# mrperkett/genome-kmers

Hardware: AMD Instinct MI355X
Metric: sorted 31-mers/sec end-to-end on 3.1 Gb synthetic genome; % HBM roofline (higher is better)
Workload: dtype u64

## Files before the change

genome-kmers_amd/csrc/gkm_msd.hip:

```cpp
#include <algorithm>
#include <cstdio>
#include <cstdlib>
#include <cstring>

#include "gkm_canon.h"
#include "gkm_internal.h"
#include "gkm_msd_config.h"
#include "gkm_partition.h"
#include "gkm_swar.h"

namespace gkm {

__constant__ uint8_t c_code4_msd[256];
static bool g_msd_tables = false;

static hipError_t msd_tables() {
    if (g_msd_tables) return hipSuccess;
    uint8_t code4[256] = {0};
    const char *order = "ABCDGHKMNRSTVWY";
    for (int i = 0; order[i]; ++i) code4[(uint8_t)order[i]] = (uint8_t)(i + 1);
    hipError_t e = hipMemcpyToSymbol(HIP_SYMBOL(c_code4_msd), code4, 256);
    if (e == hipSuccess) g_msd_tables = true;
    return e;
}
// ... 42 lines not shown
}

static unsigned resident_per_cu(gk_ctx *c, const void *fn, int threads) {
    auto it = c->occupancy.find({fn, threads});
    if (it != c->occupancy.end()) return (unsigned)it->second;
    int per_cu = 0;
    if (hipOccupancyMaxActiveBlocksPerMultiprocessor(&per_cu, fn, threads, 0) != hipSuccess || per_cu < 1)
        return 1;
    c->occupancy[{fn, threads}] = per_cu;
    return (unsigned)per_cu;
}


static bool no_compact() { return opt("GKM_NO_COMPACT") != nullptr; }

hipError_t launch_pack2(const uint8_t *from, uint64_t nwords, uint64_t *code, uint32_t *dol, hipStream_t s) {
    if (nwords == 0) return hipSuccess;
    hipLaunchKernelGGL(pack2_kernel<true>, dim3((unsigned)std::min<uint64_t>((nwords + 255) / 256, 65536)), dim3(256),
                       0, s, from, nwords, code, dol);
    return hipGetLastError();
}

static int pack_sequence(gk_ctx *c, const uint64_t **code, const uint32_t **dol) {
    const uint64_t nwords = (c->sba_len + kSbaPad) / 32;
    uint64_t *pc;
    uint32_t *pd;
    GK_TRY_HIP(c, scratch(c, "pk_code", nwords, &pc));
    GK_TRY_HIP(c, scratch(c, "pk_dol", nwords, &pd));
    int slot;
    timer_begin(c, "msd_pack", &slot);
    timer_units(c, slot, c->sba_len);
    hipLaunchKernelGGL(pack2_kernel<false>, dim3((unsigned)std::min<uint64_t>((nwords + 255) / 256, 65536)), dim3(256),
                       0, c->stream, c->sba, nwords, pc, pd);
    GK_TRY_HIP(c, hipGetLastError());
    timer_end(c, slot);
    *code = pc;
    *dol = pd;
    return GK_OK;
}

static const char *kLocPrefName[kLocal] = {"locp0", "locp1", "locp2", "locp3", "locp4", "locp5"};
static const char *kLocName[kLocal][2] = {{"loc0a", "loc0b"}, {"loc1a", "loc1b"}, {"loc2a", "loc2b"},
                                          {"loc3a", "loc3b"}, {"loc4a", "loc4b"}, {"loc5a", "loc5b"}};
static const char *kLocTimer[kLocal][2] = {{"msd_local_wave4", "msd_local_wave4_r"},
                                           {"msd_local_wave8", "msd_local_wave8_r"},
                                           {"msd_local_wave16", "msd_local_wave16_r"},
                                           {"msd_local_block16", "msd_local_block16_r"},
                                           {"msd_local_tiny", "msd_local_tiny_r"},
                                           {"msd_local_block32", "msd_local_block32_r"}};
static const char *kPassNames[] = {"msd_pass_l0", "msd_pass_l1", "msd_pass_l2", "msd_pass_l3",
                                   "msd_pass_l4", "msd_pass_l5", "msd_pass_l6", "msd_pass_l7"};
static const char *kPassNamesP[] = {"msd_pass_l0p", "msd_pass_l1p", "msd_pass_l2p", "msd_pass_l3p",
                                    "msd_pass_l4p", "msd_pass_l5p", "msd_pass_l6p", "msd_pass_l7p"};
static const char *kPassNamesC[] = {"msd_pass_l0c", "msd_pass_l1c", "msd_pass_l2c", "msd_pass_l3c",
                                    "msd_pass_l4c", "msd_pass_l5c", "msd_pass_l6c", "msd_pass_l7c"};

struct MsdDriver {
    gk_ctx *c;
    KeySpec ks;
    int B;
    uint64_t n = 0;
    unsigned cus, pgrid;
    int slot = -1, total_slot = -1;
    uint32_t *ctr = nullptr, h[kCtrN] = {0};
    unsigned long long *sums = nullptr, hs[kSumN] = {0};
    uint32_t *big_start[2], *big_len[2];
    uint64_t *big_pref[2];
    uint64_t *loc_pref[kLocal];
    uint32_t *dn_start, *dn_len;
    uint8_t *dn_par;
    uint2 *loc[kLocal][2];
    int wsched[kMaxLevels];
    int width(int level) const { return wsched[std::min(level, kMaxLevels - 1)]; }
    uint8_t *heads = nullptr;
    uint8_t *nd = nullptr;
    enum class Fmt { KeyStart, KeyStartDigit, Pairs, Compact, PackedL0 };
    Fmt cur_fmt = Fmt::KeyStart;
    int compact_hi = 0;
    bool allow_c79 = false;
    bool p88 = false;
    int p88_shi = 0;
    uint16_t *lo16_l0 = nullptr;
    uint8_t *nd_l0 = nullptr;
    int c79_shi = 0;
    uint16_t *lo16 = nullptr;
    uint32_t *tile_hist, *chunk_hist, *c_first, *c_ntiles, *seg_base, *seg_cnt;
    uint64_t nloc[kLocal] = {0}, loc_elems[kLocal] = {0}, ndone = 0, big_elems = 0;
    uint32_t nbig = 0;
    int cur_big = 0;
    int phase = 0;
    uint32_t ctiles = kChunkTiles;
    int wkeys = 0;
    L0Args l0a{};
    uint64_t l0_tiles = 0;

    MsdDriver(gk_ctx *c_, const KeySpec &ks_) : c(c_), ks(ks_), B(ks_.total_bits) {
        cus = cu_count(c);
        pgrid = cus * 4;
        set_widths(opt("GKM_LEVEL_BITS"));
        if (const char *e = opt("GKM_TEST_CHUNK_TILES")) ctiles = (uint32_t)std::max(1, std::atoi(e));
    }

    void enable_wide_l0() {
        const char *e = opt("GKM_WIDE_L0");
        const bool want = e && *e && std::strcmp(e, "0") != 0;
        if (want && ks.bits == 2 && !ks.canonical && !ks.acgt_only && B > kWideL0 + 8) wsched[0] = kWideL0;
    }

    void set_widths(const char *spec) {
        for (int l = 0; l < kMaxLevels; ++l) wsched[l] = kGR;
        if (ks.bits == 2) wsched[0] = 7;
        if (!spec) return;
        int l = 0, w = kGR;
        for (const char *p = spec; *p && l < kMaxLevels;) {
            w = std::min(8, std::max(6, std::atoi(p)));
            wsched[l++] = w;
            while (*p && *p != ',') ++p;
            if (*p == ',') ++p;
        }
        for (; l < kMaxLevels; ++l) wsched[l] = w;
        if (ks.bits != 2) wsched[0] = kGR;
        wsched[0] = std::max(wsched[0], ks.canonical ? 7 : 6);
    }

    Lists lists(int g, int bigsel) {
        return Lists{big_start[bigsel], big_len[bigsel], dn_start, dn_len, dn_par,
                     {loc[0][g], loc[1][g], loc[2][g], loc[3][g], loc[4][g], loc[5][g]}, big_pref[bigsel],
                     {g ? nullptr : loc_pref[0], g ? nullptr : loc_pref[1], g ? nullptr : loc_pref[2],
                      g ? nullptr : loc_pref[3], g ? nullptr : loc_pref[4], g ? nullptr : loc_pref[5]}};
    }

    int grow_done(uint64_t extra) {
        GK_TRY_HIP(c, grow_keep(c, "dn_start", ndone + extra, ndone, &dn_start));
        GK_TRY_HIP(c, grow_keep(c, "dn_len", ndone + extra, ndone, &dn_len));
        GK_TRY_HIP(c, grow_keep(c, "dn_par", ndone + extra, ndone, &dn_par));
        return GK_OK;
    }

    int init(uint64_t n_) {
        n = n_;
        GK_TRY_HIP(c, msd_tables());
        static_assert(4 * kCtrN <= 64 && 64 + 8 * kSumN <= 8 * kHostPinWords, "list counter block");
        uint64_t *cs;
        GK_TRY_HIP(c, scratch(c, "msd_ctr_sums", 8 + kSumN, &cs));
        ctr = reinterpret_cast<uint32_t *>(cs);
        sums = reinterpret_cast<unsigned long long *>(cs + 8);
        GK_TRY_HIP(c, hipMemsetAsync(ctr, 0, 4 * kCtrN, c->stream));
        const uint64_t max_big = n / kBlockMax + 2;
        GK_TRY_HIP(c, scratch(c, "big_start0", max_big, &big_start[0]));
        GK_TRY_HIP(c, scratch(c, "big_len0", max_big, &big_len[0]));
        GK_TRY_HIP(c, scratch(c, "big_start1", max_big, &big_start[1]));
        GK_TRY_HIP(c, scratch(c, "big_len1", max_big, &big_len[1]));
        GK_TRY_HIP(c, scratch(c, "big_pref0", max_big, &big_pref[0]));
        GK_TRY_HIP(c, scratch(c, "big_pref1", max_big, &big_pref[1]));
        if (int rc = grow_done(1024)) return rc;
        for (int k = 0; k < kLocal; ++k) GK_TRY_HIP(c, grow_keep(c, kLocName[k][0], 1024, 0, &loc[k][0]));
        for (int k = 0; k < kLocal; ++k) GK_TRY_HIP(c, grow_keep(c, kLocPrefName[k], 1024, 0, &loc_pref[k]));
        GK_TRY_HIP(c, scratch(c, "msd_heads", n + 64, &heads));
        return GK_OK;
    }

    int symbols_per_word() const { return 64 / ks.bits; }
    int phases() const { return (ks.symbols + symbols_per_word() - 1) / symbols_per_word(); }

    static constexpr uint64_t kInitLater = ~0ull;
    int begin(uint64_t n_, int key_bits = 0) {
        B = key_bits ? key_bits : ks.bits * std::min(ks.symbols, symbols_per_word());
// ... 314 lines not shown
    int classify(uint64_t nsub, int hi, int parity, int bigsel, const uint32_t *base = nullptr,
                 const uint32_t *cnt = nullptr, uint32_t min_size = 1, const uint64_t *ppref = nullptr, int pw = 0,
                 int compact = 0, bool read = true) {
        if (!base) base = seg_base;
        if (!cnt) cnt = seg_cnt;
        for (int k = 0; k < kLocal; ++k)
            GK_TRY_HIP(c, grow_keep(c, kLocName[k][0], nloc[k] + nsub, nloc[k], &loc[k][0]));
        for (int k = 0; k < kLocal; ++k)
            GK_TRY_HIP(c, grow_keep(c, kLocPrefName[k], nloc[k] + nsub, nloc[k], &loc_pref[k]));
        if (int rc = grow_done(nsub)) return rc;
        GK_TRY_HIP(c, hipMemsetAsync(ctr + kCtrBig, 0, 4, c->stream));
        GK_TRY_HIP(c, hipMemsetAsync(sums, 0, 8 * kSumN, c->stream));
        timer_begin(c, "msd_classify", &slot);
        hipLaunchKernelGGL(classify_kernel, dim3((unsigned)((nsub + kClassT - 1) / kClassT)), dim3(kClassT), 0,
                           c->stream, base, cnt, nsub, hi, B, parity, lists(0, bigsel), ctr, sums, min_size, ppref, pw,
                           compact, (uint32_t)kPTile, ctiles);
        GK_TRY_HIP(c, hipGetLastError());
        timer_end(c, slot);
        return read ? classify_counts() : GK_OK;
    }

    int classify_counts() {
        int r = read_ctr();
        if (r != GK_OK) return r;
        for (int k = 0; k < kLocal; ++k) {
            nloc[k] = h[kCtrLoc + k];
            loc_elems[k] += hs[kCtrLoc + k];
        }
        ndone = h[kCtrDone];
        nbig = h[kCtrBig];
        big_elems = hs[kCtrBig];
        return GK_OK;
    }

    int route_uniform(int out, uint32_t nb, bool dev_count) {
        const uint32_t *nb_dev = dev_count ? ctr + kCtrBig : nullptr;
        uint32_t *nb_copy = dev_count ? ctr + kCtrNbCopy : nullptr;
        const unsigned split = bucket_split(nb);
        if (dev_count && cur_fmt == Fmt::Compact)
            hipLaunchKernelGGL(expand_compact_kernel, dim3(nb, split), dim3(256), 0, c->stream, big_start[cur_big],
                               big_len[cur_big], big_pref[cur_big], compact_hi, B, nd, c->keys[out], c->vals[out],
                               nb_dev);
        uint32_t *mixed;
        GK_TRY_HIP(c, scratch(c, "uni_mixed", nb, &mixed));
        GK_TRY_HIP(c, hipMemsetAsync(mixed, 0, 4ull * nb, c->stream));
        hipLaunchKernelGGL(uniform_flag_kernel, dim3(nb, split), dim3(256), 0, c->stream, big_start[cur_big],
                           big_len[cur_big], c->keys[out], mixed, nb_dev, nb_copy);
        if (!dev_count)
            if (int rc = grow_done(nb)) return rc;
        GK_TRY_HIP(c, hipMemsetAsync(ctr + kCtrBig, 0, 4, c->stream));
        GK_TRY_HIP(c, hipMemsetAsync(sums + kCtrBig, 0, 8, c->stream));
        GK_TRY_HIP(c, hipMemsetAsync(sums + kSumTiles, 0, 16, c->stream));
        hipLaunchKernelGGL(route_uniform_kernel, dim3(grid256_min1(nb)), dim3(256), 0, c->stream, big_start[cur_big],
                           big_len[cur_big], big_pref[cur_big], nb, mixed, lists(0, cur_big ^ 1), out, ctr, sums,
                           (uint32_t)kPTile, ctiles, nb_copy);
        GK_TRY_HIP(c, hipGetLastError());
        cur_big ^= 1;
        if (dev_count) return classify_counts();
        int r = read_ctr();
        if (r != GK_OK) return r;
        ndone = h[kCtrDone];
        nbig = h[kCtrBig];
        big_elems = hs[kCtrBig];
        return GK_OK;
    }

    bool few_big_elems(int level, uint64_t elems) const {
        return level >= 1 && elems * 64 <= std::max<uint64_t>(c->n, 1);
    }

    static bool reads(Fmt in, Fmt out) {
        switch (in) {
        case Fmt::Pairs: return out == Fmt::Compact;
        case Fmt::PackedL0: return out == Fmt::Pairs;
        default: return true;
        }
    }
    bool has_digits() const { return cur_fmt != Fmt::KeyStart; }

    template <int R>
    void level_launch(int hi, int nw, const uint32_t *t_start, const uint32_t *t_count, uint64_t T,
                      const uint64_t *kin, const uint32_t *vin, int out, bool count, Fmt ofmt) {
        if (count) {
            if (has_digits())
                hipLaunchKernelGGL(msd_count_nd_kernel<R>, dim3((unsigned)T), dim3(256), 0, c->stream, t_start,
                                   t_count, nd, tile_hist);
            else
                hipLaunchKernelGGL(msd_count_kernel<R>, dim3((unsigned)T), dim3(256), 0, c->stream, t_start, t_count,
                                   dig_at(B, hi, R), kin, tile_hist);
            return;
        }
        if (ofmt == Fmt::Compact) {
            const int rem = B - hi - R;
            NextDigits ndg{dig_at(B, hi + R, 8), nd};
            ndg.lowmask = (uint32_t)((1ull << (rem - 8)) - 1);
            if (cur_fmt == Fmt::Pairs)
                hipLaunchKernelGGL((msd_pipe_kernel<kPT, kPI, R, 4, true, 0, true>), dim3(pgrid), dim3(kPT), 0,
                                   c->stream, t_start, t_count, dig_at(B, hi, R), tile_hist, kin, vin, c->keys[out],
                                   c->vals[out], (uint32_t)T, n, ndg, lo16, c79_shi);
            else
                hipLaunchKernelGGL((msd_pipe_kernel<kPT, kPI, R, 4, true>), dim3(pgrid), dim3(kPT), 0, c->stream,
                                   t_start, t_count, dig_at(B, hi, R), tile_hist, kin, vin, c->keys[out],
                                   c->vals[out], (uint32_t)T, n, ndg);
            return;
        }
        if (ofmt == Fmt::Pairs) {
            NextDigits ndg{dig_at(B, hi + R, nw), nd};
            ndg.out16 = lo16;
            ndg.pshi = c79_shi;
            if (cur_fmt == Fmt::PackedL0) {
                ndg.in8 = nd_l0;
                hipLaunchKernelGGL((msd_pipe_kernel<kPT, kPI, R, 5, true, 0, 2>), dim3(pgrid), dim3(kPT), 0, c->stream,
                                   t_start, t_count, dig_at(B, hi, R), tile_hist, kin, vin, c->keys[out], c->vals[out],
                                   (uint32_t)T, n, ndg, lo16_l0, p88_shi);
                return;
            }
            hipLaunchKernelGGL((msd_pipe_kernel<kPT, kPI, R, 5, true>), dim3(pgrid), dim3(kPT), 0, c->stream, t_start,
                               t_count, dig_at(B, hi, R), tile_hist, kin, vin, c->keys[out], c->vals[out],
                               (uint32_t)T, n, ndg);
            return;
        }
        const NextDigits ndg{dig_at(B, hi + R, nw), nd};
        if (ofmt == Fmt::KeyStartDigit)
            hipLaunchKernelGGL((msd_pipe_kernel<kPT, kPI, R, 0, true>), dim3(pgrid), dim3(kPT), 0, c->stream, t_start,
                               t_count, dig_at(B, hi, R), tile_hist, kin, vin, c->keys[out], c->vals[out],
                               (uint32_t)T, n, ndg);
        else
            hipLaunchKernelGGL((msd_pipe_kernel<kPT, kPI, R, 0, false>), dim3(pgrid), dim3(kPT), 0, c->stream,
                               t_start, t_count, dig_at(B, hi, R), tile_hist, kin, vin, c->keys[out], c->vals[out],
                               (uint32_t)T, n, ndg);
    }

    void level_dispatch(int level, int hi, const uint32_t *t_start, const uint32_t *t_count, uint64_t T,
                        const uint64_t *kin, const uint32_t *vin, int out, bool count, Fmt ofmt) {
        const int w = width(level), nw = width(level + 1);
        if (w == 8) level_launch<8>(hi, nw, t_start, t_count, T, kin, vin, out, count, ofmt);
        else if (w == 7) level_launch<7>(hi, nw, t_start, t_count, T, kin, vin, out, count, ofmt);
        else level_launch<6>(hi, nw, t_start, t_count, T, kin, vin, out, count, ofmt);
    }

    Fmt level_format(int level, int hi, uint64_t elems, uint64_t nseg) const {
        const bool digits = nseg == 0 || (elems / nseg >> width(level)) >= (uint64_t)kBlockMax;
        const int rem = B - hi - width(level);
        if (phase == 0 && !digits && rem >= 9 && rem <= 40 && width(level + 1) == 8 && !no_compact())
            return Fmt::Compact;
        const uint64_t next_mean = nseg ? (elems / nseg >> width(level)) >> width(level + 1) : 0;
        const int rem2 = rem - width(level + 1);
        const bool force = opt("GKM_TEST_PAIRS") != nullptr;
        if (allow_c79 && cur_fmt != Fmt::Pairs && phase == 0 && rem >= 33 && rem <= 48 && !no_compact() &&
            (force || (digits && next_mean < (uint64_t)kBlockMax && rem2 >= 9 && rem2 <= 40 &&
                       width(level + 2) == 8 && width(level + 1) == 8)))
            return Fmt::Pairs;
        return digits ? Fmt::KeyStartDigit : Fmt::KeyStart;
    }

    int level_pass(int level, int hi, const uint32_t *t_start, const uint32_t *t_count, uint64_t T, uint64_t C,
                   const uint32_t *s_cfirst, const uint32_t *s_nchunks, const uint32_t *s_start, uint64_t nseg,
                   const uint64_t *kin, const uint32_t *vin, int out) {
        timer_begin(c, has_digits() ? "msd_count_nd" : "msd_count", &slot);
        timer_units(c, slot, big_elems);
        level_dispatch(level, hi, t_start, t_count, T, kin, vin, out, true, cur_fmt);
        GK_TRY_HIP(c, hipGetLastError());
        timer_end(c, slot);
        int rc = scan_offsets(width(level), C, s_cfirst, s_nchunks, s_start, nseg);
        if (rc != GK_OK) return rc;
        GK_TRY_HIP(c, scratch(c, "msd_nd", n + 64, &nd));
        const Fmt ofmt = level_format(level, hi, big_elems, nseg);
        compact_hi = hi + width(level);
        const int rem = B - hi - width(level);
        if (ofmt == Fmt::Pairs) {
            c79_shi = 64 - rem;
            GK_TRY_HIP(c, scratch(c, "msd_lo16", n + 64, &lo16));
        }
        if (!reads(cur_fmt, ofmt)) {
            if (cur_fmt == Fmt::PackedL0) {
                if (int rc = p88_detach()) return rc;
                hipLaunchKernelGGL(expand_p88_kernel, dim3((unsigned)nseg, bucket_split(nseg)), dim3(256), 0,
                                   c->stream, big_start[cur_big], big_len[cur_big], big_pref[cur_big], hi, B, p88_shi,
                                   const_cast<uint64_t *>(kin), lo16_l0, nd_l0, const_cast<uint32_t *>(vin));
            } else {
                hipLaunchKernelGGL(expand_pair_kernel, dim3((unsigned)nseg, bucket_split(nseg)), dim3(256), 0,
                                   c->stream, big_start[cur_big], big_len[cur_big], big_pref[cur_big], hi, B, c79_shi,
                                   const_cast<uint64_t *>(kin), lo16, const_cast<uint32_t *>(vin));
            }
            GK_TRY_HIP(c, hipGetLastError());
            cur_fmt = Fmt::KeyStartDigit;
        }
        timer_begin(c, ofmt == Fmt::Compact ? kPassNamesC[level & 7] : ofmt == Fmt::Pairs ? kPassNamesP[level & 7]
                                                                                          : kPassNames[level & 7],
                    &slot);
        timer_units(c, slot, big_elems);
        level_dispatch(level, hi, t_start, t_count, T, kin, vin, out, false, ofmt);
        GK_TRY_HIP(c, hipGetLastError());
        timer_end(c, slot);
        cur_fmt = ofmt;
        return GK_OK;
    }

    int expand_pair_locals(const uint64_t (&before)[kLocal], int out) {
        for (int k = 0; k < kLocal; ++k) {
            if (nloc[k] <= before[k]) continue;
            hipLaunchKernelGGL(expand_pair_list_kernel, dim3((unsigned)(nloc[k] - before[k])), dim3(256), 0,
                               c->stream, loc[k][0], loc_pref[k], (uint32_t)before[k], B, c79_shi, c->keys[out], lo16,
                               c->vals[out]);
            GK_TRY_HIP(c, hipGetLastError());
        }
        return GK_OK;
    }

    int first_level_from_pieces(const uint64_t *kin, const uint32_t *vin, const uint64_t *poff, const uint64_t *plen,
                                const uint32_t *pbucket, uint32_t np, int level = 1, int hi = kGR) {
        std::vector<uint32_t> ts, tc, cf, cn, scf, snc, sst;
        std::vector<uint64_t> spf;
        uint64_t out_base = 0;
        for (uint32_t i = 0; i < np;) {
            uint32_t j = i;
            uint64_t tot = 0;
            const uint64_t tile0 = ts.size();
            while (j < np && pbucket[j] == pbucket[i]) {
                for (uint64_t o = 0; o < plen[j]; o += kPTile) {
                    ts.push_back((uint32_t)(poff[j] + o));
                    tc.push_back((uint32_t)std::min<uint64_t>(kPTile, plen[j] - o));
                }
                tot += plen[j];
                ++j;
            }
            if (tot > 0) {
                const uint64_t nt = ts.size() - tile0;
                scf.push_back((uint32_t)cf.size());
                for (uint64_t t = 0; t < nt; t += ctiles) {
                    cf.push_back((uint32_t)(tile0 + t));
                    cn.push_back((uint32_t)std::min<uint64_t>(ctiles, nt - t));
                }
                snc.push_back((uint32_t)(cf.size() - scf.back()));
                sst.push_back((uint32_t)out_base);
                spf.push_back(pbucket[i]);
                out_base += tot;
            }
            i = j;
        }
        if (out_base != n) return fail(c, GK_E_ARG, "piece lengths do not add up to n");
        const uint64_t T = ts.size(), C = cf.size(), nseg = sst.size();
        if (nseg == 0) return GK_OK;
        int rc = tables(T, C, nseg);
        if (rc != GK_OK) return rc;
        uint32_t *t_start, *t_count, *s_cfirst, *s_nchunks, *s_st;
        GK_TRY_HIP(c, scratch(c, "t_start", T, &t_start));
        GK_TRY_HIP(c, scratch(c, "t_count", T, &t_count));
        GK_TRY_HIP(c, scratch(c, "s_cfirst", nseg, &s_cfirst));
        GK_TRY_HIP(c, scratch(c, "s_nchunks", nseg, &s_nchunks));
        GK_TRY_HIP(c, scratch(c, "s_pstart", nseg, &s_st));
        GK_TRY_HIP(c, hipMemcpyAsync(t_start, ts.data(), 4 * T, hipMemcpyHostToDevice, c->stream));
        GK_TRY_HIP(c, hipMemcpyAsync(t_count, tc.data(), 4 * T, hipMemcpyHostToDevice, c->stream));
        GK_TRY_HIP(c, hipMemcpyAsync(c_first, cf.data(), 4 * C, hipMemcpyHostToDevice, c->stream));
        GK_TRY_HIP(c, hipMemcpyAsync(c_ntiles, cn.data(), 4 * C, hipMemcpyHostToDevice, c->stream));
        GK_TRY_HIP(c, hipMemcpyAsync(s_cfirst, scf.data(), 4 * nseg, hipMemcpyHostToDevice, c->stream));
        GK_TRY_HIP(c, hipMemcpyAsync(s_nchunks, snc.data(), 4 * nseg, hipMemcpyHostToDevice, c->stream));
        GK_TRY_HIP(c, hipMemcpyAsync(s_st, sst.data(), 4 * nseg, hipMemcpyHostToDevice, c->stream));
        uint64_t *s_pref;
        GK_TRY_HIP(c, scratch(c, "s_ppref", nseg, &s_pref));
        GK_TRY_HIP(c, hipMemcpyAsync(s_pref, spf.data(), 8 * nseg, hipMemcpyHostToDevice, c->stream));
        GK_TRY_HIP(c, hipStreamSynchronize(c->stream));
        big_elems = n;
        if (!reads(cur_fmt, level_format(level, hi, n, nseg))) {
            if (int rd = p88_detach()) return rd;
            uint64_t *pdev;
            GK_TRY_HIP(c, scratch(c, "p88_pieces", 3 * np, &pdev));
            std::vector<uint64_t> hp(3 * (uint64_t)np);
            for (uint32_t j = 0; j < np; ++j) {
                hp[j] = poff[j];
                hp[np + j] = plen[j];
                hp[2 * (uint64_t)np + j] = pbucket[j];
            }
            GK_TRY_HIP(c, hipMemcpyAsync(pdev, hp.data(), 8 * hp.size(), hipMemcpyHostToDevice, c->stream));
            hipLaunchKernelGGL(expand_p88_pieces_kernel, dim3(np, bucket_split(np)), dim3(256), 0, c->stream, pdev,
                               np, hi, B, p88_shi, const_cast<uint64_t *>(kin), lo16_l0, nd_l0,
                               const_cast<uint32_t *>(vin));
            GK_TRY_HIP(c, hipGetLastError());
            GK_TRY_HIP(c, hipStreamSynchronize(c->stream));
            cur_fmt = Fmt::KeyStartDigit;
        }
        rc = level_pass(level, hi, t_start, t_count, T, C, s_cfirst, s_nchunks, s_st, nseg, kin, vin, 0);
        if (rc != GK_OK) return rc;
        cur_big = 0;
        uint64_t before[kLocal];
        for (int k = 0; k < kLocal; ++k) before[k] = nloc[k];
// ... 807 lines not shown
```

genome-kmers_amd/csrc/gkm_msd_lists.h:

```cpp
#pragma once

#include <hip/hip_runtime.h>
#include <stdint.h>

#include "gkm_msd_config.h"
#include "gkm_msd_scan.h"
#include "gkm_partition.h"

namespace gkm {

__device__ __forceinline__ uint32_t wave_append(bool flag, uint32_t *counter, int lane) {
    const uint64_t m = __ballot(flag);
    if (!m) return 0;
    const int leader = __ffsll((unsigned long long)m) - 1;
    uint32_t base = 0;
    if (lane == leader) base = atomicAdd(counter, (uint32_t)__popcll(m));
    base = __shfl(base, leader);
    const uint64_t lt_mask = (lane == 0) ? 0ull : (~0ull >> (64 - lane));
    return base + (uint32_t)__popcll(m & lt_mask);
}

enum { kCtrBig = 0, kCtrDone = 1, kCtrLoc = 2, kLists = kCtrLoc + kLocal, kCtrNbCopy = kLists, kCtrN = 8 + 2 };
enum { kSumTiles = kLists, kSumChunks = kLists + 1, kSumN = kLists + 2 };

// ... 56 lines not shown

__global__ __launch_bounds__(kClassT) void classify_kernel(const uint32_t *__restrict__ seg_base,
                                                           const uint32_t *__restrict__ seg_cnt, uint64_t nsub, int hi,
                                                           int B, int parity, Lists L, uint32_t *__restrict__ ctr,
                                                           unsigned long long *__restrict__ sums, uint32_t min_size,
                                                           const uint64_t *__restrict__ ppref, int pw, int compact,
                                                           uint32_t tile, uint32_t ctiles) {
    constexpr int NW = kClassT / 64;
    __shared__ uint32_t s_cnt[kLists][NW];
    __shared__ uint32_t s_elems[kLists][NW];
    __shared__ uint32_t s_base[kLists];
    __shared__ uint32_t s_tc[2][NW];
    const int tid = threadIdx.x, lane = tid & 63, wave = tid >> 6;
    const uint64_t i = (uint64_t)blockIdx.x * kClassT + tid;
    const uint32_t size = i < nsub ? seg_cnt[i] : 0, st = i < nsub ? seg_base[i] : 0;
    const int li = size >= min_size ? list_of(size, hi, B, true) : -1;
    bool f[kLists];
#pragma unroll
    for (int l = 0; l < kLists; ++l) f[l] = li == l;
    uint32_t below[kLists];
#pragma unroll
    for (int l = 0; l < kLists; ++l) {
        const uint64_t m = __ballot(f[l]);
        below[l] = lanes_below(m);
        uint32_t e = f[l] ? size : 0;
#pragma unroll
        for (int off = 32; off >= 1; off >>= 1) e += __shfl_xor(e, off);
        if (lane == 0) {
            s_cnt[l][wave] = (uint32_t)__popcll(m);
            s_elems[l][wave] = e;
        }
    }
    {
        uint32_t tl = li == kCtrBig ? tiles_of(size, tile) : 0, ch = li == kCtrBig ? chunks_of(size, tile, ctiles) : 0;
#pragma unroll
        for (int off = 32; off >= 1; off >>= 1) {
            tl += __shfl_xor(tl, off);
            ch += __shfl_xor(ch, off);
        }
        if (lane == 0) {
            s_tc[0][wave] = tl;
            s_tc[1][wave] = ch;
        }
    }
    __syncthreads();
    if (tid >= 64 && tid < 66) {
        unsigned long long t = 0;
        for (int w = 0; w < NW; ++w) t += s_tc[tid - 64][w];
        if (t) atomicAdd(&sums[kSumTiles + tid - 64], t);
    }
    if (tid < kLists) {
        uint32_t tot = 0;
        unsigned long long el = 0;
        for (int w = 0; w < NW; ++w) {
            tot += s_cnt[tid][w];
            el += s_elems[tid][w];
        }
        s_base[tid] = tot ? atomicAdd(&ctr[tid], tot) : 0;
        if (el) atomicAdd(&sums[tid], el);
    }
    __syncthreads();
    uint32_t at[kLists];
#pragma unroll
    for (int l = 0; l < kLists; ++l) {
        uint32_t pre = s_base[l];
        for (int w = 0; w < wave; ++w) pre += s_cnt[l][w];
        at[l] = pre + below[l];
    }
    uint64_t pref = 0;
    if (li >= 0) {
        if (pw > 0) pref = ((ppref ? ppref[i >> pw] & ~kCompact : 0ull) << pw) | (i & ((1ull << pw) - 1));
        else pref = ppref ? ppref[i] & ~kCompact : 0ull;
        if (compact) pref |= kCompact;
    }
#pragma unroll
    for (int l = 0; l < kLists; ++l)
        if (li == l) put_entry(L, l, at[l], st, size, hi, parity, pref);
}

static unsigned bucket_split(uint64_t nbuckets) { return nbuckets <= 4096 ? 32u : nbuckets <= 65536 ? 4u : 1u; }

__global__ __launch_bounds__(256) void expand_pair_kernel(const uint32_t *__restrict__ bst,
                                                          const uint32_t *__restrict__ blen,
                                                          const uint64_t *__restrict__ bpref, int hi, int B, int shi,
                                                          uint64_t *__restrict__ kio, const uint16_t *__restrict__ in16,
                                                          uint32_t *__restrict__ vout) {
    const uint64_t st = bst[blockIdx.x];
    const uint32_t len = blen[blockIdx.x];
    const uint64_t top = (bpref[blockIdx.x] & ~kCompact) << (B - hi);
    for (uint32_t e = blockIdx.y * 256 + threadIdx.x; e < len; e += gridDim.y * 256) {
        uint64_t key;
        uint32_t val;
        unpack_pair(kio[st + e], in16[st + e], shi, key, val);
        kio[st + e] = top | key;
        vout[st + e] = val;
    }
}

__global__ __launch_bounds__(256) void expand_pair_list_kernel(const uint2 *__restrict__ list,
                                                               const uint64_t *__restrict__ pref, uint32_t first,
                                                               int B, int shi, uint64_t *__restrict__ kio,
                                                               const uint16_t *__restrict__ in16,
                                                               uint32_t *__restrict__ vout) {
    const uint2 en = list[first + blockIdx.x];
    const uint64_t st = en.x;
    const uint32_t len = en.y >> 8;
    const int hi = (en.y >> 1) & 127;
    const uint64_t top = (pref[first + blockIdx.x] & ~kCompact) << (B - hi);
    for (uint32_t e = threadIdx.x; e < len; e += 256) {
        uint64_t key;
        uint32_t val;
        unpack_pair(kio[st + e], in16[st + e], shi, key, val);
        kio[st + e] = top | key;
        vout[st + e] = val;
    }
}

__device__ __forceinline__ void unpack_p88(uint64_t a, uint32_t lo, uint32_t dg, int shi, uint64_t &rel, uint32_t &val) {
    unpack_pair(a, lo, shi, rel, val);
    rel |= (uint64_t)dg << (64 - shi);
}

__global__ __launch_bounds__(256) void expand_p88_kernel(const uint32_t *__restrict__ bst,
                                                         const uint32_t *__restrict__ blen,
                                                         const uint64_t *__restrict__ bpref, int hi, int B, int shi,
                                                         uint64_t *__restrict__ kio, const uint16_t *__restrict__ in16,
                                                         const uint8_t *__restrict__ in8, uint32_t *__restrict__ vout) {
    const uint64_t st = bst[blockIdx.x];
    const uint32_t len = blen[blockIdx.x];
    const uint64_t top = (bpref[blockIdx.x] & ~kCompact) << (B - hi);
    for (uint32_t e = blockIdx.y * 256 + threadIdx.x; e < len; e += gridDim.y * 256) {
        uint64_t rel;
        uint32_t val;
        unpack_p88(kio[st + e], in16[st + e], in8[st + e], shi, rel, val);
        kio[st + e] = top | rel;
        vout[st + e] = val;
    }
}

__global__ __launch_bounds__(256) void expand_p88_list_kernel(const uint2 *__restrict__ list,
                                                              const uint64_t *__restrict__ pref, int B, int shi,
                                                              uint64_t *__restrict__ kio, const uint16_t *__restrict__ in16,
                                                              const uint8_t *__restrict__ in8,
                                                              uint32_t *__restrict__ vout) {
    const uint2 en = list[blockIdx.x];
    const uint64_t st = en.x;
    const uint32_t len = en.y >> 8;
    const int hi = (en.y >> 1) & 127;
    const uint64_t top = (pref[blockIdx.x] & ~kCompact) << (B - hi);
    for (uint32_t e = threadIdx.x; e < len; e += 256) {
        uint64_t rel;
        uint32_t val;
        unpack_p88(kio[st + e], in16[st + e], in8[st + e], shi, rel, val);
        kio[st + e] = top | rel;
        vout[st + e] = val;
    }
}

__global__ __launch_bounds__(256) void expand_p88_pieces_kernel(const uint64_t *__restrict__ pp, uint32_t np, int hi,
                                                                int B, int shi, uint64_t *__restrict__ kio,
                                                                const uint16_t *__restrict__ in16,
                                                                const uint8_t *__restrict__ in8,
                                                                uint32_t *__restrict__ vout) {
    const uint64_t st = pp[blockIdx.x], len = pp[np + blockIdx.x];
    const uint64_t top = pp[2 * (uint64_t)np + blockIdx.x] << (B - hi);
    for (uint64_t e = blockIdx.y * 256 + threadIdx.x; e < len; e += gridDim.y * 256) {
        uint64_t rel;
        uint32_t val;
        unpack_p88(kio[st + e], in16[st + e], in8[st + e], shi, rel, val);
        kio[st + e] = top | rel;
        vout[st + e] = val;
    }
}

__global__ __launch_bounds__(256) void expand_compact_kernel(const uint32_t *__restrict__ bst,
                                                             const uint32_t *__restrict__ blen,
                                                             const uint64_t *__restrict__ bpref, int hi, int B,
                                                             const uint8_t *__restrict__ nd,
                                                             uint64_t *__restrict__ kio, uint32_t *__restrict__ vout,
                                                             const uint32_t *__restrict__ nb_dev = nullptr) {
    if (nb_dev && blockIdx.x >= *nb_dev) return;
    const uint64_t st = bst[blockIdx.x];
    const uint32_t len = blen[blockIdx.x];
    const uint64_t pf = bpref[blockIdx.x];
    for (uint32_t e = blockIdx.y * 256 + threadIdx.x; e < len; e += gridDim.y * 256) {
        const uint64_t x = kio[st + e];
        kio[st + e] = compact_key(pf, hi, B, nd[st + e], (uint32_t)(x >> 32));
        vout[st + e] = (uint32_t)x;
    }
}

__global__ void lists_store_kernel(Lists L, Lists *__restrict__ dst) { *dst = L; }

__global__ __launch_bounds__(256) void uniform_flag_kernel(const uint32_t *__restrict__ bst,
                                                           const uint32_t *__restrict__ blen,
                                                           const uint64_t *__restrict__ keys,
                                                           uint32_t *__restrict__ mixed,
                                                           const uint32_t *__restrict__ nb_dev = nullptr,
                                                           uint32_t *__restrict__ nb_copy = nullptr) {
    if (nb_copy && blockIdx.x == 0 && blockIdx.y == 0 && threadIdx.x == 0) *nb_copy = *nb_dev;
    if (nb_dev && blockIdx.x >= *nb_dev) return;
    const uint64_t st = bst[blockIdx.x];
// ... 46 lines not shown
```

genome-kmers_amd/csrc/gkm_partition.h:

```cpp
#pragma once

#include <hip/hip_runtime.h>
#include <stdint.h>

namespace gkm {

template <class T>
__device__ __forceinline__ __attribute__((address_space(1))) T *gmem(T *p) {
    return (__attribute__((address_space(1))) T *)p;
}
typedef __attribute__((address_space(1))) const uint64_t gu64;
typedef __attribute__((address_space(1))) const uint8_t gu8;
typedef __attribute__((address_space(1))) const uint32_t __attribute__((aligned(1))) gu32u;

__device__ __forceinline__ void lds_barrier() {
    __builtin_amdgcn_fence(__ATOMIC_RELEASE, "workgroup", "local");
    __builtin_amdgcn_s_barrier();
    __builtin_amdgcn_fence(__ATOMIC_ACQUIRE, "workgroup", "local");
}

constexpr int kVmcnt0 = 0x0F70;
constexpr int vmcnt_imm(int v) { return kVmcnt0 | (v & 15) | ((v >> 4) << 14); }

struct Dig {
    int shift;
    uint32_t mask;
};

__host__ __device__ inline Dig dig_at(int B, int hi, int w) {
    if (hi >= B) return Dig{0, 0u};
    int lo = B - hi - w;
    if (lo < 0) lo = 0;
    return Dig{lo, (uint32_t)((1ull << (B - hi - lo)) - 1)};
}

__device__ __forceinline__ uint32_t dg_of(uint64_t k, Dig d) { return (uint32_t)(k >> d.shift) & d.mask; }

__host__ __device__ inline uint2 local_entry(uint32_t start, uint32_t len, int hi, int parity) {
    return make_uint2(start, (len << 8) | ((uint32_t)hi << 1) | (uint32_t)parity);
}

__device__ __forceinline__ uint32_t lanes_below(uint64_t m) {
    return __builtin_amdgcn_mbcnt_hi((uint32_t)(m >> 32), __builtin_amdgcn_mbcnt_lo((uint32_t)m, 0u));
}

static __constant__ int g_rank_ballot = 0;

template <int DB = 10, bool P16 = false>
__device__ __forceinline__ uint32_t rank_ballot(uint32_t *wc, uint32_t d, bool valid) {
    uint64_t m = __ballot(valid);
#pragma unroll
    for (int b = 0; b < DB; ++b) {
        const uint64_t x = __ballot((d >> b) & 1u);
        m &= ((d >> b) & 1u) ? x : ~x;
    }
    const uint32_t below = lanes_below(m);
    uint32_t old = 0;
    if (valid && below == 0) {
        if (P16) {
            const uint32_t sh = (d & 1u) << 4;
            old = (atomicAdd(&wc[d >> 1], (uint32_t)__popcll(m) << sh) >> sh) & 0xFFFFu;
        } else {
            old = atomicAdd(&wc[d], (uint32_t)__popcll(m));
        }
    }
    const int leader = m ? __builtin_ctzll(m) : 0;
    old = (uint32_t)__builtin_amdgcn_ds_bpermute(leader << 2, (int)old);
    return valid ? old + below : 0u;
}

__device__ __forceinline__ uint32_t rank_atomic(uint32_t *wc, uint32_t d, bool valid) {
    if (__builtin_expect(g_rank_ballot != 0, 0)) return rank_ballot(wc, d, valid);
    return valid ? atomicAdd(&wc[d], 1u) : 0u;
}

template <int DB = 11>
__device__ __forceinline__ uint32_t rank_atomic16(uint32_t *wc, uint32_t d, bool valid) {
    if (__builtin_expect(g_rank_ballot != 0, 0)) return rank_ballot<DB, true>(wc, d, valid);
    const uint32_t sh = (d & 1u) << 4;
    return valid ? (atomicAdd(&wc[d >> 1], 1u << sh) >> sh) & 0xFFFFu : 0u;
}

static inline hipError_t set_rank_ballot_here(int on) {
    return hipMemcpyToSymbol(HIP_SYMBOL(g_rank_ballot), &on, sizeof(int));
}

// ... 138 lines not shown
        for (int g = 0; g < G; ++g) o[g] = s_toff[dg_of(k[g], d)] + s[g];
#pragma unroll
        for (int g = 0; g < G; ++g) {
            uint64_t oo = cnt ? (uint64_t)o[g] : sink;
            if (MODE == 3) oo = seq_base + s[g];
            if (MODE != 1 || oo == 0xFFFFFFFFu) {
                kout[oo] = k[g];
                vout[oo] = v[g];
            }
        }
    }
}

struct TileWalk {
    uint32_t first, end, step;
    __device__ TileWalk(uint32_t ntiles) {
        const uint32_t x = blockIdx.x & 7, per = gridDim.x >> 3;
        first = (uint32_t)((uint64_t)ntiles * x / 8) + (blockIdx.x >> 3);
        end = (uint32_t)((uint64_t)ntiles * (x + 1) / 8);
        step = per;
    }
};

template <int R>
__global__ __launch_bounds__(256) void msd_count_kernel(const uint32_t *__restrict__ t_start,
                                                        const uint32_t *__restrict__ t_count, Dig dl,
                                                        const uint64_t *__restrict__ kin,
                                                        uint32_t *__restrict__ tile_hist) {
    constexpr int RADIX = 1 << R;
    __shared__ uint32_t s_hist[RADIX];
    const int t = threadIdx.x;
    for (int i = t; i < RADIX; i += 256) s_hist[i] = 0;
    lds_barrier();
    const uint64_t b = t_start[blockIdx.x];
    const uint32_t m = t_count[blockIdx.x];
    for (uint32_t i = t; i < m; i += 256) atomicAdd(&s_hist[dg_of(kin[b + i], dl)], 1u);
    lds_barrier();
    for (int i = t; i < RADIX; i += 256) tile_hist[(uint64_t)blockIdx.x * RADIX + i] = s_hist[i];
}

template <int R>
__global__ __launch_bounds__(256) void msd_count_nd_kernel(const uint32_t *__restrict__ t_start,
                                                           const uint32_t *__restrict__ t_count,
                                                           const uint8_t *__restrict__ nd,
                                                           uint32_t *__restrict__ tile_hist) {
    constexpr int RADIX = 1 << R;
#ifndef GKM_COUNT_COPIES
#define GKM_COUNT_COPIES 1
#endif
    constexpr int NC = GKM_COUNT_COPIES;
    __shared__ uint32_t s_hist[RADIX * NC];
    const int t = threadIdx.x;
    for (int i = t; i < RADIX * NC; i += 256) s_hist[i] = 0;
    lds_barrier();
    uint32_t *hc = s_hist + (t & (NC - 1));
    const uint64_t b = t_start[blockIdx.x];
    const uint32_t m = t_count[blockIdx.x];
    const uint32_t head = min<uint32_t>((uint32_t)((16 - ((uintptr_t)(nd + b) & 15)) & 15), m);
    const uint32_t quads = (m - head) >> 4;
    const uint4 *w = reinterpret_cast<const uint4 *>(nd + b + head);
    if (t < (int)head) atomicAdd(&hc[NC * nd[b + t]], 1u);
    for (uint32_t i0 = 0; i0 < quads; i0 += 3 * 256) {
        uint4 x4[3];
#pragma unroll
        for (int r = 0; r < 3; ++r) {
            const uint32_t i = i0 + r * 256 + t;
            x4[r] = i < quads ? w[i] : make_uint4(0, 0, 0, 0);
        }
#pragma unroll
        for (int r = 0; r < 3; ++r) {
            if (i0 + r * 256 + t >= quads) continue;
            const uint32_t xs[4] = {x4[r].x, x4[r].y, x4[r].z, x4[r].w};
#pragma unroll
            for (int u = 0; u < 4; ++u) {
                atomicAdd(&hc[NC * (xs[u] & 0xFF)], 1u);
                atomicAdd(&hc[NC * ((xs[u] >> 8) & 0xFF)], 1u);
                atomicAdd(&hc[NC * ((xs[u] >> 16) & 0xFF)], 1u);
                atomicAdd(&hc[NC * (xs[u] >> 24)], 1u);
            }
        }
    }
    const uint32_t tail0 = head + 16 * quads;
    if (tail0 + t < m) atomicAdd(&hc[NC * nd[b + tail0 + t]], 1u);
    lds_barrier();
    for (int i = t; i < RADIX; i += 256) {
        uint32_t v = 0;
#pragma unroll
        for (int c = 0; c < NC; ++c) v += s_hist[NC * i + c];
        tile_hist[(uint64_t)blockIdx.x * RADIX + i] = v;
    }
}

template <int T, int I, int R, int MODE = 0, bool PROF = false>
__global__ __launch_bounds__(T) void msd_scatter_kernel(const uint32_t *__restrict__ t_start,
                                                        const uint32_t *__restrict__ t_count, Dig dl,
                                                        const uint32_t *__restrict__ tile_off,
                                                        const uint64_t *__restrict__ kin,
                                                        const uint32_t *__restrict__ vin, uint64_t *__restrict__ kout,
                                                        uint32_t *__restrict__ vout, uint32_t ntiles,
                                                        uint64_t sink, unsigned long long *prof = nullptr,
                                                        int stagger = 0) {
    using SM = PartSmem<T, I, R>;
    constexpr int RADIX = SM::kRadix;
    __shared__ __attribute__((aligned(16))) unsigned char s_raw[SM::kUnion];
    __shared__ uint32_t s_toff[RADIX];
    __shared__ uint32_t s_wsum[SM::kWaves];
    __shared__ uint32_t s_start[RADIX + 1];
    const int tid = threadIdx.x, lane = tid & 63, wave = tid >> 6;
    uint32_t *s_wc = reinterpret_cast<uint32_t *>(s_raw);
    const TileWalk walk(ntiles);
    uint64_t key[I];
    uint32_t val[I], m = 0, toff = 0;
    auto load = [&](uint32_t t) {
        const uint64_t b = t_start[t];
        m = t_count[t];
        toff = tile_off[(uint64_t)t * RADIX + (tid & (RADIX - 1))];
        uint32_t q0 = wave * (I * 64) + lane;
        asm volatile("" : "+v"(q0));
#pragma unroll
        for (int i = 0; i < I; ++i) {
            const uint64_t e = b + min(q0 + i * 64, m - 1);
            key[i] = kin[e];
            val[i] = vin[e];
        }
    };
    if (stagger && blockIdx.x >= gridDim.x / 2)
        for (int i = 0; i < stagger; ++i) __builtin_amdgcn_s_sleep(127);
    if (walk.first < walk.end) load(walk.first);
    __builtin_amdgcn_s_waitcnt(kVmcnt0);
    uint64_t tp = PROF ? clock64() : 0;
    for (uint32_t t = walk.first; t < walk.end; t += walk.step) {
        lds_barrier();
        if (PROF && tid == 0) {
            const uint64_t t1 = clock64();
            atomicAdd(&prof[5], (unsigned long long)(t1 - tp));
            tp = t1;
        }
        for (int i = tid; i < SM::kWaves * RADIX; i += T) s_wc[i] = 0;
        if (tid < RADIX) s_toff[tid] = toff;
        lds_barrier();
        if (PROF && tid == 0) {
            const uint64_t t1 = clock64();
            atomicAdd(&prof[4], (unsigned long long)(t1 - tp));
            tp = t1;
        }
        bool valid[I];
#pragma unroll
        for (int i = 0; i < I; ++i) valid[i] = (uint32_t)(wave * (I * 64) + i * 64 + lane) < m;
        uint32_t slot[I];
        partition_stage<T, I, R, PROF>(key, val, valid, dl, s_raw, s_toff, s_wsum, s_start, slot, prof);
        if (PROF) tp = clock64();
        const uint32_t cnt = s_start[RADIX];
        const uint64_t seq = (uint64_t)t * (T * I);
        if (t + walk.step < walk.end) load(t + walk.step);
        partition_store<T, I, R, MODE>(dl, s_raw, s_toff, cnt, sink, kout, vout, seq);
    }
}

template <int T, int I>
struct PipeSmem {
    static constexpr int kTile = T * I;
    static constexpr int kWaves = T / 64;
    static constexpr int kValOff = (kTile + 2) * 8;
    static constexpr int kStage = kValOff + (kTile + 1) * 4;
};

struct NextDigits {
    Dig d;
    uint8_t *out;
    uint32_t lowmask = 0;
    uint16_t *out16 = nullptr;
    int pshi = 0;
    const uint8_t *in8 = nullptr;
};

__device__ __forceinline__ void unpack_pair(uint64_t a, uint32_t b16, int shi, uint64_t &key, uint32_t &val) {
    key = a >> shi;
    val = ((uint32_t)(a & ((1ull << shi) - 1)) << (32 - shi)) | b16;
}

template <int T, int I, int R, int MODE, bool ND>
__device__ __forceinline__ void pipe_store(int g, Dig d, const uint64_t *s_keys, const uint32_t *s_vals,
                                           const uint32_t *toff, uint32_t cnt, uint64_t sink,
                                           uint64_t *__restrict__ kout, uint32_t *__restrict__ vout,
                                           NextDigits nd, uint32_t base = 0) {
    const uint32_t s = min((uint32_t)(threadIdx.x + g * T), cnt - 1);
    const uint64_t k = s_keys[s];
    const uint32_t v = s_vals[s];
    const uint64_t o = cnt ? (uint64_t)(toff[dg_of(k, d)] + base + s) : sink;
    if (MODE == 4) {
        kout[o] = ((uint64_t)((uint32_t)k & nd.lowmask) << 32) | v;
        nd.out[o] = (uint8_t)dg_of(k, nd.d);
    } else if (MODE == 5) {
        const int shi = nd.pshi;
        kout[o] = ((k & ((1ull << (64 - shi)) - 1)) << shi) | (v >> (32 - shi));
        nd.out16[o] = (uint16_t)(v & ((1u << (32 - shi)) - 1));
        nd.out[o] = (uint8_t)dg_of(k, nd.d);
    } else if (MODE != 1 || o == 0xFFFFFFFFu) {
        kout[o] = k;
        vout[o] = v;
        if (ND) nd.out[o] = (uint8_t)dg_of(k, nd.d);
    }
}

template <int T, int I, int R = 8, int MODE = 0, bool ND = false, int PRE_ = 0, int INP = 0>
__global__ __launch_bounds__(T) void msd_pipe_kernel(const uint32_t *__restrict__ t_start,
                                                     const uint32_t *__restrict__ t_count, Dig dl,
                                                     const uint32_t *__restrict__ tile_off,
                                                     const uint64_t *__restrict__ kin, const uint32_t *__restrict__ vin,
                                                     uint64_t *__restrict__ kout, uint32_t *__restrict__ vout,
                                                     uint32_t ntiles, uint64_t sink, NextDigits nd = {},
                                                     const uint16_t *__restrict__ in16 = nullptr, int in_shi = 0) {
    static_assert(INP == 0 || MODE == 4 || MODE == 5, "packed-pair input keeps only the unsorted key bits");
    using SM = PipeSmem<T, I>;
    constexpr int NW = SM::kWaves;
    constexpr int TILE = SM::kTile;
    constexpr int PRE = PRE_ ? PRE_ : (I + 2) / 3;
    constexpr int RADIX = 1 << R;
    static_assert(T >= RADIX, "one thread per digit");
    __shared__ __attribute__((aligned(16))) unsigned char s_stage[SM::kStage];
    __shared__ uint32_t s_wc[NW * RADIX];
    __shared__ uint32_t s_toff[2][RADIX];
    __shared__ uint32_t s_start[RADIX + 1];
    __shared__ uint32_t s_wsum[RADIX / 64 > 0 ? RADIX / 64 : 1];
    uint64_t *s_keys = reinterpret_cast<uint64_t *>(s_stage);
    uint32_t *s_vals = reinterpret_cast<uint32_t *>(s_stage + SM::kValOff);
    const int tid = threadIdx.x, lane = tid & 63, wave = tid >> 6;
    const TileWalk walk(ntiles);
    uint64_t key[I];
    uint32_t val[I], m = 0, toff = 0;
    auto load = [&](uint32_t t) {
        toff = tile_off[(uint64_t)t * RADIX + (tid & (RADIX - 1))];
        const uint64_t b = t_start[t];
        m = t_count[t];
        uint32_t q0 = wave * (I * 64) + lane;
        asm volatile("" : "+v"(q0));
#pragma unroll
        for (int i = 0; i < I; ++i) {
            const uint64_t e = b + min(q0 + i * 64, m - 1);
            if (INP == 1) {
                key[i] = kin[e];
                val[i] = in16[e];
            } else if (INP == 2) {
                key[i] = kin[e];
                val[i] = in16[e] | ((uint32_t)nd.in8[e] << 16);
            } else {
                key[i] = kin[e];
                val[i] = vin[e];
            }
        }
    };
    uint32_t pcnt = 0;
    int cur = 0;
    if (walk.first < walk.end) load(walk.first);
    __builtin_amdgcn_s_waitcnt(kVmcnt0);
    for (uint32_t t = walk.first; t < walk.end; t += walk.step) {
        uint32_t *wc = s_wc + wave * RADIX;
#pragma unroll
        for (int u = 0; u < (RADIX + 63) / 64; ++u)
            if (u * 64 + lane < RADIX) wc[u * 64 + lane] = 0;
        if (tid < RADIX) s_toff[cur][tid] = toff;
        const uint32_t *ptoff = s_toff[cur ^ 1];
#pragma unroll
        for (int g = 0; g < PRE; ++g) pipe_store<T, I, R, MODE, ND>(g, dl, s_keys, s_vals, ptoff, pcnt, sink, kout, vout, nd);
        bool valid[I];
        uint32_t dig[I], rank[I];
#pragma unroll
        for (int i = 0; i < I; ++i) {
            valid[i] = (uint32_t)(wave * (I * 64) + i * 64 + lane) < m;
            if (INP == 1) unpack_pair(key[i], val[i], in_shi, key[i], val[i]);
            if (INP == 2) {
                const uint64_t top = (uint64_t)(val[i] >> 16) << (64 - in_shi);
                unpack_pair(key[i], val[i] & 0xFFFFu, in_shi, key[i], val[i]);
                key[i] |= top;
            }
            dig[i] = dg_of(key[i], dl);
            rank[i] = rank_atomic(wc, dig[i], valid[i]);
            if (PRE + i < I) pipe_store<T, I, R, MODE, ND>(PRE + i, dl, s_keys, s_vals, ptoff, pcnt, sink, kout, vout, nd);
        }
        lds_barrier();
        uint32_t total = 0, incl = 0;
        if (tid < RADIX) {
#pragma unroll
            for (int w = 0; w < NW; ++w) {
                const uint32_t v = s_wc[w * RADIX + tid];
                s_wc[w * RADIX + tid] = total;
                total += v;
            }
            incl = wave_incl_scan(total);
            if (lane == 63) s_wsum[wave] = incl;
        }
        lds_barrier();
        if (tid < RADIX) {
            uint32_t pre = 0;
            for (int w = 0; w < wave; ++w) pre += s_wsum[w];
            const uint32_t st = pre + incl - total;
            s_start[tid] = st;
            s_toff[cur][tid] -= st;
            if (tid == RADIX - 1) s_start[RADIX] = pre + incl;
        }
        lds_barrier();
#pragma unroll
        for (int i = 0; i < I; ++i) {
            const uint32_t sl = valid[i] ? s_start[dig[i]] + wc[dig[i]] + rank[i] : (uint32_t)TILE;
            s_keys[sl] = key[i];
            s_vals[sl] = val[i];
        }
        pcnt = s_start[RADIX];
        lds_barrier();
        if (t + walk.step < walk.end) load(t + walk.step);
        cur ^= 1;
    }
    if (walk.first < walk.end) {
        const uint32_t *ptoff = s_toff[cur ^ 1];
#pragma unroll
        for (int g = 0; g < I; ++g) pipe_store<T, I, R, MODE, ND>(g, dl, s_keys, s_vals, ptoff, pcnt, sink, kout, vout, nd);
    }
}

}
```

Measured before the change: 44.62 billion.

## Embed next-level digit in packed pair high bits, dropping separate nd array

```diff
diff --git a/genome-kmers_amd/csrc/gkm_msd.hip b/genome-kmers_amd/csrc/gkm_msd.hip
--- a/genome-kmers_amd/csrc/gkm_msd.hip
+++ b/genome-kmers_amd/csrc/gkm_msd.hip
@@ -148,7 +148,7 @@
     int p88_shi = 0;
     uint16_t *lo16_l0 = nullptr;
     uint8_t *nd_l0 = nullptr;
-    int c79_shi = 0;
+    PairFmt c79_fmt{};
     uint16_t *lo16 = nullptr;
     uint32_t *tile_hist, *chunk_hist, *c_first, *c_ntiles, *seg_base, *seg_cnt;
     uint64_t nloc[kLocal] = {0}, loc_elems[kLocal] = {0}, ndone = 0, big_elems = 0;
@@ -629,7 +629,10 @@
     void level_launch(int hi, int nw, const uint32_t *t_start, const uint32_t *t_count, uint64_t T,
                       const uint64_t *kin, const uint32_t *vin, int out, bool count, Fmt ofmt) {
         if (count) {
-            if (has_digits())
+            if (cur_fmt == Fmt::Pairs)
+                hipLaunchKernelGGL(msd_count_pair_kernel<R>, dim3((unsigned)T), dim3(256), 0, c->stream, t_start,
+                                   t_count, lo16, tile_hist);
+            else if (has_digits())
                 hipLaunchKernelGGL(msd_count_nd_kernel<R>, dim3((unsigned)T), dim3(256), 0, c->stream, t_start,
                                    t_count, nd, tile_hist);
             else
@@ -644,7 +647,7 @@
             if (cur_fmt == Fmt::Pairs)
                 hipLaunchKernelGGL((msd_pipe_kernel<kPT, kPI, R, 4, true, 0, true>), dim3(pgrid), dim3(kPT), 0,
                                    c->stream, t_start, t_count, dig_at(B, hi, R), tile_hist, kin, vin, c->keys[out],
-                                   c->vals[out], (uint32_t)T, n, ndg, lo16, c79_shi);
+                                   c->vals[out], (uint32_t)T, n, ndg, lo16, 0, c79_fmt);
             else
                 hipLaunchKernelGGL((msd_pipe_kernel<kPT, kPI, R, 4, true>), dim3(pgrid), dim3(kPT), 0, c->stream,
                                    t_start, t_count, dig_at(B, hi, R), tile_hist, kin, vin, c->keys[out],
@@ -652,9 +655,9 @@
             return;
         }
         if (ofmt == Fmt::Pairs) {
-            NextDigits ndg{dig_at(B, hi + R, nw), nd};
+            NextDigits ndg{dig_at(B, hi + R, nw), nullptr};
             ndg.out16 = lo16;
-            ndg.pshi = c79_shi;
+            ndg.pf = c79_fmt;
             if (cur_fmt == Fmt::PackedL0) {
                 ndg.in8 = nd_l0;
                 hipLaunchKernelGGL((msd_pipe_kernel<kPT, kPI, R, 5, true, 0, 2>), dim3(pgrid), dim3(kPT), 0, c->stream,
@@ -711,14 +714,10 @@
         timer_end(c, slot);
         int rc = scan_offsets(width(level), C, s_cfirst, s_nchunks, s_start, nseg);
         if (rc != GK_OK) return rc;
-        GK_TRY_HIP(c, scratch(c, "msd_nd", n + 64, &nd));
         const Fmt ofmt = level_format(level, hi, big_elems, nseg);
         compact_hi = hi + width(level);
         const int rem = B - hi - width(level);
-        if (ofmt == Fmt::Pairs) {
-            c79_shi = 64 - rem;
-            GK_TRY_HIP(c, scratch(c, "msd_lo16", n + 64, &lo16));
-        }
+        if (ofmt != Fmt::Pairs) GK_TRY_HIP(c, scratch(c, "msd_nd", n + 64, &nd));
         if (!reads(cur_fmt, ofmt)) {
             if (cur_fmt == Fmt::PackedL0) {
                 if (int rc = p88_detach()) return rc;
@@ -727,11 +726,15 @@
                                    const_cast<uint64_t *>(kin), lo16_l0, nd_l0, const_cast<uint32_t *>(vin));
             } else {
                 hipLaunchKernelGGL(expand_pair_kernel, dim3((unsigned)nseg, bucket_split(nseg)), dim3(256), 0,
-                                   c->stream, big_start[cur_big], big_len[cur_big], big_pref[cur_big], hi, B, c79_shi,
-                                   const_cast<uint64_t *>(kin), lo16, const_cast<uint32_t *>(vin));
+                                   c->stream, big_start[cur_big], big_len[cur_big], big_pref[cur_big], hi, B, c79_fmt,
+                                   const_cast<uint64_t *>(kin), lo16, const_cast<uint32_t *>(vin), nd);
             }
             GK_TRY_HIP(c, hipGetLastError());
             cur_fmt = Fmt::KeyStartDigit;
+        }
+        if (ofmt == Fmt::Pairs) {
+            c79_fmt = pair_fmt(rem, width(level + 1));
+            GK_TRY_HIP(c, scratch(c, "msd_lo16", n + 64, &lo16));
         }
         timer_begin(c, ofmt == Fmt::Compact ? kPassNamesC[level & 7] : ofmt == Fmt::Pairs ? kPassNamesP[level & 7]
                                                                                           : kPassNames[level & 7],
@@ -748,7 +751,7 @@
         for (int k = 0; k < kLocal; ++k) {
             if (nloc[k] <= before[k]) continue;
             hipLaunchKernelGGL(expand_pair_list_kernel, dim3((unsigned)(nloc[k] - before[k])), dim3(256), 0,
-                               c->stream, loc[k][0], loc_pref[k], (uint32_t)before[k], B, c79_shi, c->keys[out], lo16,
+                               c->stream, loc[k][0], loc_pref[k], (uint32_t)before[k], B, c79_fmt, c->keys[out], lo16,
                                c->vals[out]);
             GK_TRY_HIP(c, hipGetLastError());
         }
diff --git a/genome-kmers_amd/csrc/gkm_msd_lists.h b/genome-kmers_amd/csrc/gkm_msd_lists.h
--- a/genome-kmers_amd/csrc/gkm_msd_lists.h
+++ b/genome-kmers_amd/csrc/gkm_msd_lists.h
@@ -162,24 +162,26 @@
 
 __global__ __launch_bounds__(256) void expand_pair_kernel(const uint32_t *__restrict__ bst,
                                                           const uint32_t *__restrict__ blen,
-                                                          const uint64_t *__restrict__ bpref, int hi, int B, int shi,
+                                                          const uint64_t *__restrict__ bpref, int hi, int B, PairFmt f,
                                                           uint64_t *__restrict__ kio, const uint16_t *__restrict__ in16,
-                                                          uint32_t *__restrict__ vout) {
+                                                          uint32_t *__restrict__ vout, uint8_t *__restrict__ nd_out) {
     const uint64_t st = bst[blockIdx.x];
     const uint32_t len = blen[blockIdx.x];
     const uint64_t top = (bpref[blockIdx.x] & ~kCompact) << (B - hi);
     for (uint32_t e = blockIdx.y * 256 + threadIdx.x; e < len; e += gridDim.y * 256) {
         uint64_t key;
         uint32_t val;
-        unpack_pair(kio[st + e], in16[st + e], shi, key, val);
+        const uint32_t b = in16[st + e];
+        unpack_pair(f, kio[st + e], b, key, val);
         kio[st + e] = top | key;
         vout[st + e] = val;
+        nd_out[st + e] = (uint8_t)pair_digit(b, f.nw);
     }
 }
 
 __global__ __launch_bounds__(256) void expand_pair_list_kernel(const uint2 *__restrict__ list,
                                                                const uint64_t *__restrict__ pref, uint32_t first,
-                                                               int B, int shi, uint64_t *__restrict__ kio,
+                                                               int B, PairFmt f, uint64_t *__restrict__ kio,
                                                                const uint16_t *__restrict__ in16,
                                                                uint32_t *__restrict__ vout) {
     const uint2 en = list[first + blockIdx.x];
@@ -190,14 +192,14 @@
     for (uint32_t e = threadIdx.x; e < len; e += 256) {
         uint64_t key;
         uint32_t val;
-        unpack_pair(kio[st + e], in16[st + e], shi, key, val);
+        unpack_pair(f, kio[st + e], in16[st + e], key, val);
         kio[st + e] = top | key;
         vout[st + e] = val;
     }
 }
 
 __device__ __forceinline__ void unpack_p88(uint64_t a, uint32_t lo, uint32_t dg, int shi, uint64_t &rel, uint32_t &val) {
-    unpack_pair(a, lo, shi, rel, val);
+    unpack_l0_pair(a, lo, shi, rel, val);
     rel |= (uint64_t)dg << (64 - shi);
 }
 
diff --git a/genome-kmers_amd/csrc/gkm_pair_format.h b/genome-kmers_amd/csrc/gkm_pair_format.h
--- /dev/null
+++ b/genome-kmers_amd/csrc/gkm_pair_format.h
@@ -0,0 +1,37 @@
+#pragma once
+
+#include <stdint.h>
+
+#if defined(__HIPCC__)
+#define GKM_PAIR_HD __host__ __device__ __forceinline__
+#else
+#define GKM_PAIR_HD inline
+#endif
+
+namespace gkm {
+
+struct PairFmt {
+    int nkb;
+    int lowb;
+    int nw;
+};
+
+GKM_PAIR_HD PairFmt pair_fmt(int rem, int nw) {
+    const int nkb = rem - nw;
+    return PairFmt{nkb, nkb > 32 ? nkb - 32 : 0, nw};
+}
+
+GKM_PAIR_HD uint32_t pair_digit(uint32_t b, int nw) { return b >> (16 - nw); }
+
+GKM_PAIR_HD void pack_pair(PairFmt f, uint64_t key, uint32_t start, uint64_t &a, uint16_t &b) {
+    const uint32_t dig = (uint32_t)(key >> f.nkb) & ((1u << f.nw) - 1);
+    a = ((key & ((1ull << f.nkb) - 1)) << (32 - f.lowb)) | (start >> f.lowb);
+    b = (uint16_t)((dig << (16 - f.nw)) | (start & ((1u << f.lowb) - 1)));
+}
+
+GKM_PAIR_HD void unpack_pair(PairFmt f, uint64_t a, uint32_t b, uint64_t &key, uint32_t &start) {
+    key = ((uint64_t)pair_digit(b, f.nw) << f.nkb) | (a >> (32 - f.lowb));
+    start = ((uint32_t)a << f.lowb) | (b & ((1u << f.lowb) - 1));
+}
+
+}
diff --git a/genome-kmers_amd/csrc/gkm_partition.h b/genome-kmers_amd/csrc/gkm_partition.h
--- a/genome-kmers_amd/csrc/gkm_partition.h
+++ b/genome-kmers_amd/csrc/gkm_partition.h
@@ -2,6 +2,8 @@
 
 #include <hip/hip_runtime.h>
 #include <stdint.h>
+
+#include "gkm_pair_format.h"
 
 namespace gkm {
 
@@ -306,6 +308,53 @@
     }
     const uint32_t tail0 = head + 16 * quads;
     if (tail0 + t < m) atomicAdd(&hc[NC * nd[b + tail0 + t]], 1u);
+    lds_barrier();
+    for (int i = t; i < RADIX; i += 256) {
+        uint32_t v = 0;
+#pragma unroll
+        for (int c = 0; c < NC; ++c) v += s_hist[NC * i + c];
+        tile_hist[(uint64_t)blockIdx.x * RADIX + i] = v;
+    }
+}
+
+template <int R>
+__global__ __launch_bounds__(256) void msd_count_pair_kernel(const uint32_t *__restrict__ t_start,
+                                                             const uint32_t *__restrict__ t_count,
+                                                             const uint16_t *__restrict__ lo16,
+                                                             uint32_t *__restrict__ tile_hist) {
+    constexpr int RADIX = 1 << R;
+    constexpr int NC = GKM_COUNT_COPIES;
+    __shared__ uint32_t s_hist[RADIX * NC];
+    const int t = threadIdx.x;
+    for (int i = t; i < RADIX * NC; i += 256) s_hist[i] = 0;
+    lds_barrier();
+    uint32_t *hc = s_hist + (t & (NC - 1));
+    const uint64_t b = t_start[blockIdx.x];
+    const uint32_t m = t_count[blockIdx.x];
+    const uint32_t head = min<uint32_t>((uint32_t)(((16 - ((uintptr_t)(lo16 + b) & 15)) & 15) >> 1), m);
+    const uint32_t octs = (m - head) >> 3;
+    const uint4 *w = reinterpret_cast<const uint4 *>(lo16 + b + head);
+    if (t < (int)head) atomicAdd(&hc[NC * pair_digit(lo16[b + t], R)], 1u);
+    for (uint32_t i0 = 0; i0 < octs; i0 += 3 * 256) {
+        uint4 x4[3];
+#pragma unroll
+        for (int r = 0; r < 3; ++r) {
+            const uint32_t i = i0 + r * 256 + t;
+            x4[r] = i < octs ? w[i] : make_uint4(0, 0, 0, 0);
+        }
+#pragma unroll
+        for (int r = 0; r < 3; ++r) {
+            if (i0 + r * 256 + t >= octs) continue;
+            const uint32_t xs[4] = {x4[r].x, x4[r].y, x4[r].z, x4[r].w};
+#pragma unroll
+            for (int u = 0; u < 4; ++u) {
+                atomicAdd(&hc[NC * pair_digit(xs[u] & 0xFFFFu, R)], 1u);
+                atomicAdd(&hc[NC * pair_digit(xs[u] >> 16, R)], 1u);
+            }
+        }
+    }
+    const uint32_t tail0 = head + 8 * octs;
+    if (tail0 + t < m) atomicAdd(&hc[NC * pair_digit(lo16[b + tail0 + t], R)], 1u);
     lds_barrier();
     for (int i = t; i < RADIX; i += 256) {
         uint32_t v = 0;
@@ -395,10 +444,11 @@
     uint32_t lowmask = 0;
     uint16_t *out16 = nullptr;
     int pshi = 0;
+    PairFmt pf{};
     const uint8_t *in8 = nullptr;
 };
 
-__device__ __forceinline__ void unpack_pair(uint64_t a, uint32_t b16, int shi, uint64_t &key, uint32_t &val) {
+__device__ __forceinline__ void unpack_l0_pair(uint64_t a, uint32_t b16, int shi, uint64_t &key, uint32_t &val) {
     key = a >> shi;
     val = ((uint32_t)(a & ((1ull << shi) - 1)) << (32 - shi)) | b16;
 }
@@ -416,10 +466,11 @@
         kout[o] = ((uint64_t)((uint32_t)k & nd.lowmask) << 32) | v;
         nd.out[o] = (uint8_t)dg_of(k, nd.d);
     } else if (MODE == 5) {
-        const int shi = nd.pshi;
-        kout[o] = ((k & ((1ull << (64 - shi)) - 1)) << shi) | (v >> (32 - shi));
-        nd.out16[o] = (uint16_t)(v & ((1u << (32 - shi)) - 1));
-        nd.out[o] = (uint8_t)dg_of(k, nd.d);
+        uint64_t a;
+        uint16_t b;
+        pack_pair(nd.pf, k, v, a, b);
+        kout[o] = a;
+        nd.out16[o] = b;
     } else if (MODE != 1 || o == 0xFFFFFFFFu) {
         kout[o] = k;
         vout[o] = v;
@@ -434,7 +485,8 @@
                                                      const uint64_t *__restrict__ kin, const uint32_t *__restrict__ vin,
                                                      uint64_t *__restrict__ kout, uint32_t *__restrict__ vout,
                                                      uint32_t ntiles, uint64_t sink, NextDigits nd = {},
-                                                     const uint16_t *__restrict__ in16 = nullptr, int in_shi = 0) {
+                                                     const uint16_t *__restrict__ in16 = nullptr, int in_shi = 0,
+                                                     PairFmt in_pf = {}) {
     static_assert(INP == 0 || MODE == 4 || MODE == 5, "packed-pair input keeps only the unsorted key bits");
     using SM = PipeSmem<T, I>;
     constexpr int NW = SM::kWaves;
@@ -492,10 +544,10 @@
 #pragma unroll
         for (int i = 0; i < I; ++i) {
             valid[i] = (uint32_t)(wave * (I * 64) + i * 64 + lane) < m;
-            if (INP == 1) unpack_pair(key[i], val[i], in_shi, key[i], val[i]);
+            if (INP == 1) unpack_pair(in_pf, key[i], val[i], key[i], val[i]);
             if (INP == 2) {
                 const uint64_t top = (uint64_t)(val[i] >> 16) << (64 - in_shi);
-                unpack_pair(key[i], val[i] & 0xFFFFu, in_shi, key[i], val[i]);
+                unpack_l0_pair(key[i], val[i] & 0xFFFFu, in_shi, key[i], val[i]);
                 key[i] |= top;
             }
             dig[i] = dg_of(key[i], dl);
```

Result: faster. 45.29 billion (median of 6 runs) (+1.5%).
